# mihikamd/DP-GSAT

Measured on AMD Instinct MI355X. Metric: million edges/s (attn+sample+aggregate fwd+bwd), higher is better.
Workload: dtype f32

## Files before the change

### dp_gsat_amd/csrc/pna.hip

```cpp
#include "common.h"
#include "pna_math.h"

namespace gsat {

constexpr int PNA_BLOCK = 128;
constexpr int SC_AMP = GSAT_SCALE_AMPLIFICATION, SC_ATT = GSAT_SCALE_ATTENUATION, SC_LIN = GSAT_SCALE_LINEAR, SC_INVLIN = GSAT_SCALE_INVERSE_LINEAR;

struct PnaCfg {
    int A, S;
    int aggr[8];
    int scal[8];
    float avg_lin, avg_log;
};

__device__ __forceinline__ int pna_xcd_remap(int b, int nb) {
    int q = nb >> 3, r = nb & 7, x = b & 7, i = b >> 3;
    return (x < r ? x * (q + 1) : r * (q + 1) + (x - r) * q) + i;
}

__device__ __forceinline__ float scaler_factor(int s, float deg, float avg_lin, float avg_log) {
    switch (s) {
        case SC_AMP: return logf(deg + 1.f) / avg_log;
        case SC_ATT: return deg == 0.f ? 1.f : avg_log / logf(deg + 1.f);
        case SC_LIN: return deg / avg_lin;
// ... 539 lines not shown
                const int k = kb + u, e = e4[u];
                const float w = w4[u];
                const float4 xj = x4[u];
                float da = 0.f;
                if (on) {
                    float4 dm;
                    dm.x = fmaf(Qj.x, w * xj.x, Pj.x) + (k == jmin.x ? gmn_j.x : 0.f) + (k == jmax.x ? gmx_j.x : 0.f);
                    dm.y = fmaf(Qj.y, w * xj.y, Pj.y) + (k == jmin.y ? gmn_j.y : 0.f) + (k == jmax.y ? gmx_j.y : 0.f);
                    dm.z = fmaf(Qj.z, w * xj.z, Pj.z) + (k == jmin.z ? gmn_j.z : 0.f) + (k == jmax.z ? gmx_j.z : 0.f);
                    dm.w = fmaf(Qj.w, w * xj.w, Pj.w) + (k == jmin.w ? gmn_j.w : 0.f) + (k == jmax.w ? gmx_j.w : 0.f);
                    st4(dmsg + (size_t)k * H + c, f4scale(w, dm));
                    da += f4dot(dm, xj);
                    da += t1 + w * t2 + (k == kmin_a ? tmn : 0.f) + (k == kmax_a ? tmx : 0.f);
                    if (HAS_EE) {
                        const float4 ee = ee4[u];
                        float4 de;
                        de.x = fmaf(Qe.x, w * ee.x, Pe.x) + (k == emin.x ? gmn_e.x : 0.f) + (k == emax.x ? gmx_e.x : 0.f);
                        de.y = fmaf(Qe.y, w * ee.y, Pe.y) + (k == emin.y ? gmn_e.y : 0.f) + (k == emax.y ? gmx_e.y : 0.f);
                        de.z = fmaf(Qe.z, w * ee.z, Pe.z) + (k == emin.z ? gmn_e.z : 0.f) + (k == emax.z ? gmx_e.z : 0.f);
                        de.w = fmaf(Qe.w, w * ee.w, Pe.w) + (k == emin.w ? gmn_e.w : 0.f) + (k == emax.w ? gmx_e.w : 0.f);
                        if (dedge) st4(dedge + (size_t)e * H + c, f4scale(w, de));
                        da += f4dot(de, ee);
                    }
                }
                if (datt) {
                    da = group_sum<LPR>(da);
                    if (lane == 0) datt[e] = c0 ? datt[e] + da : da;
                }
            }
        }
    }
}

constexpr int TILE_BLOCK = 512;

__global__ void k_pna_tiles(const int32_t* __restrict__ node_ptr, const int32_t* __restrict__ node_seg, const int32_t* __restrict__ rowptr,
                            const int32_t* __restrict__ rowptr_src, int N, int TN, int slack, int T, int4* __restrict__ desc,
                            int32_t* __restrict__ spill_count) {
    const int t = blockIdx.x * blockDim.x + threadIdx.x;
    if (t == 0 && spill_count) *spill_count = 0;
    if (t > T) return;
    const int64_t p = (int64_t)t * TN;
    int start = N;
    if (t < T && p < N) {
        start = (int)p;
        if (node_seg) {
            const int g0 = node_ptr[node_seg[p]];
            start = min((int)p, max(g0, (int)p - slack));
        }
    }
    desc[t] = make_int4(start, rowptr[start], rowptr_src[start], 0);
}

template <int LPR, int NAGG, bool NATT>
__global__ __launch_bounds__(TILE_BLOCK, 4) void k_pna_bwd_tile(
    const float* __restrict__ x, const float* __restrict__ att, const float* __restrict__ dout, const int32_t* __restrict__ rowptr,
    const int32_t* __restrict__ col, const int32_t* __restrict__ eid, const int4* __restrict__ desc,
    const int32_t* __restrict__ rowptr_src, const int32_t* __restrict__ slot_map, int H, int TE, int RCAP, float* dx,
    float* __restrict__ dmsg, float* datt, float* __restrict__ dw, const float* __restrict__ dx_add, int datt_acc) {
    constexpr int GPB = LaneGroups<LPR, TILE_BLOCK>::GPB;
    constexpr int RPW = 64 / LPR;
    constexpr int NSEG = NAGG * 2;
    extern __shared__ float4 smem4[];
    float4* erow = smem4;
    int* s_col = reinterpret_cast<int*>(erow + (size_t)TE * LPR);
    int* s_eid = s_col + TE;
    float* s_w = reinterpret_cast<float*>(s_eid);
    float* s_att = reinterpret_cast<float*>(s_eid + TE);
    int* s_slot = reinterpret_cast<int*>(s_att + TE);
    int* s_rp = s_slot + TE;
    int* s_rps = s_rp + RCAP + 1;
    float* s_na = reinterpret_cast<float*>(s_rps + RCAP + 1);
    float* s_dna = s_na + RCAP + 1;
    const int tid = threadIdx.x, wave = tid >> 6;
    const LaneGroups<LPR, TILE_BLOCK> lg;
    const int grp = lg.grp < 0 ? GPB : lg.grp;
    const int lane = lg.lane, c = lane * 4;
    const bool on = c < H && lg.grp >= 0;
    const int t = pna_xcd_remap(blockIdx.x, gridDim.x);
    const int4 d0 = desc[t], d1 = desc[t + 1];
    const int n0 = d0.x, n1 = d1.x;
    if (n1 <= n0) return;
    const int nr = n1 - n0;
    const int k0 = d0.y, ne = min(d1.y - k0, TE);
    const int s0 = d0.z, ns = d1.z - s0, nsl = min(ns, TE);
    float4 dcur[NSEG];
    float4 xi_cur = f4zero();
    const uint32_t hb = (uint32_t)H * 4u, gb = NSEG * hb, cb = (uint32_t)c * 4u;
    const float* gwin = dout + (size_t)n0 * NSEG * H;
    const float* xwin = x + (size_t)n0 * H;
    float* dxwin = dx + (size_t)n0 * H;
    float* mwin = dmsg + (size_t)k0 * H;
    int r = lg.grp >= 0 ? grp : nr;
#pragma unroll
    for (int sg = 0; sg < NSEG; ++sg) dcur[sg] = f4zero();
    if (r < nr && on) {
#pragma unroll
        for (int sg = 0; sg < NSEG; ++sg) dcur[sg] = ld4_off(gwin, r * gb + sg * hb + cb);
        xi_cur = ld4_off(xwin, r * hb + cb);
    }
    for (int i = tid; i <= nr; i += TILE_BLOCK) {
        s_rp[i] = rowptr[n0 + i] - k0;
        s_rps[i] = rowptr_src[n0 + i] - s0;
        if (NATT) { s_na[i] = att[min(n0 + i, n1 - 1)]; s_dna[i] = 0.f; }
    }
    for (int i = tid; i < ne; i += TILE_BLOCK) {
        s_col[i] = col[k0 + i];
        if (!NATT) s_eid[i] = eid[k0 + i];
    }
    for (int i = tid; i < nsl; i += TILE_BLOCK) s_slot[i] = slot_map[s0 + i] - k0;
    __syncthreads();
    for (int base = 0; base < ne; base += GPB) {
        const int i = base + grp;
        if (i < ne && on)
            __builtin_amdgcn_global_load_lds((const __attribute__((address_space(1))) void*)(x + (size_t)s_col[i] * H + c),
                                             (__attribute__((address_space(3))) void*)(erow + (size_t)(base + wave * RPW) * LPR), 16, 0, 0);
    }
    for (int i = tid; i < ne; i += TILE_BLOCK) {
        if (NATT) {
            s_att[i] = att[s_col[i]];
        } else {
            s_att[i] = att ? att[s_eid[i]] : 1.f;
        }
    }
    asm volatile("s_waitcnt vmcnt(0)" ::: "memory");
    __syncthreads();
    float4 dx_keep = f4zero();
    for (; r < nr; r += GPB) {
        const int nr_ = r + GPB;
        const int beg = s_rp[r], end = s_rp[r + 1];
        const float na_row = NATT ? s_na[r] : 0.f;
        const float cnt = (float)(end - beg);
        float sa = 0.f, sa2 = 0.f, amin = INFINITY, amax = -INFINITY;
        int kmin_a = beg, kmax_a = beg;
        Acc4 aj;
        aj.init();
        int4 jmin = make_int4(beg, beg, beg, beg), jmax = jmin;
        float wfirst = 1.f;
        const int mid = min(end, max(beg, ne));
        auto stats = [&](int k, float w, float4 xv) {
            if (k == beg) wfirst = w;
            sa += w; sa2 = fmaf(w, w, sa2);
            if (w < amin) { amin = w; kmin_a = k; }
            if (w > amax) { amax = w; kmax_a = k; }
            const float4 m = f4scale(w, xv);
#define GSAT_TARG(C)                                                                                                       \
            if (m.C < aj.mn.C) { jmin.C = k; aj.mn.C = m.C; }                                                              \
            if (m.C > aj.mx.C) { jmax.C = k; aj.mx.C = m.C; }
            GSAT_TARG(x) GSAT_TARG(y) GSAT_TARG(z) GSAT_TARG(w)
#undef GSAT_TARG
            aj.s.x += m.x; aj.s.y += m.y; aj.s.z += m.z; aj.s.w += m.w;
            aj.q.x = fmaf(m.x, m.x, aj.q.x); aj.q.y = fmaf(m.y, m.y, aj.q.y); aj.q.z = fmaf(m.z, m.z, aj.q.z); aj.q.w = fmaf(m.w, m.w, aj.q.w);
        };
        for (int k = beg; k < mid; ++k)
            stats(k, NATT ? s_att[k] * na_row : s_att[k], on ? erow[(size_t)k * LPR + lane] : f4zero());
        for (int k = mid; k < end; ++k)
            stats(k, NATT ? att[col[k0 + k]] * na_row : (att ? att[eid[k0 + k]] : 1.f), on ? ld4(x + (size_t)col[k0 + k] * H + c) : f4zero());
        const float4 xi = xi_cur;
        const Acc4 ai = self_stats(xi, sa, sa2, amin, amax);
        const float n = fmaxf(cnt, 1.f), inv_n = 1.f / n;
        float t1 = 0.f, t2 = 0.f, tmn = 0.f, tmx = 0.f;
        float4 Pi, Qi, Pj, Qj, gmn_i, gmx_i, gmn_j, gmx_j;
#define GSAT_TFOLD(ACC, PART, P, Q, GMN, GMX)                                                                              \
        {                                                                                                                  \
            const float4 mean = f4scale(inv_n, ACC.s);                                                                     \
            const float4 var = make_float4(ACC.q.x * inv_n - mean.x * mean.x, ACC.q.y * inv_n - mean.y * mean.y,           \
                                           ACC.q.z * inv_n - mean.z * mean.z, ACC.q.w * inv_n - mean.w * mean.w);          \
            const float4 hs = make_float4(var.x > 0.f ? 0.5f * __builtin_amdgcn_rsqf(var.x + 1e-5f) : 0.f,                 \
                                          var.y > 0.f ? 0.5f * __builtin_amdgcn_rsqf(var.y + 1e-5f) : 0.f,                 \
                                          var.z > 0.f ? 0.5f * __builtin_amdgcn_rsqf(var.z + 1e-5f) : 0.f,                 \
                                          var.w > 0.f ? 0.5f * __builtin_amdgcn_rsqf(var.w + 1e-5f) : 0.f);                \
            float4 p0 = f4scale(inv_n, dcur[0 * 2 + (PART)]);                                                              \
            if (NAGG == 5) { const float4 vsum = dcur[(NAGG == 5 ? 4 : 0) * 2 + (PART)];                                   \
                             p0 = make_float4(p0.x + vsum.x, p0.y + vsum.y, p0.z + vsum.z, p0.w + vsum.w); }               \
            GMN = dcur[1 * 2 + (PART)];                                                                                    \
            GMX = dcur[2 * 2 + (PART)];                                                                                    \
            const float4 vs = dcur[3 * 2 + (PART)];                                                                        \
            const float4 gv = make_float4(vs.x * hs.x, vs.y * hs.y, vs.z * hs.z, vs.w * hs.w);                             \
            Q = f4scale(2.f * inv_n, gv);                                                                                  \
            P = make_float4(p0.x - mean.x * Q.x, p0.y - mean.y * Q.y, p0.z - mean.z * Q.z, p0.w - mean.w * Q.w);           \
        }
        GSAT_TFOLD(ai, 0, Pi, Qi, gmn_i, gmx_i)
        if (on) {
            float4 dxi;
#define GSAT_TSELF(C)                                                                                                      \
            {                                                                                                              \
                const float xc = xi.C;                                                                                     \
                const float wlo = xc > 0.f ? amin : (xc < 0.f ? amax : wfirst), whi = xc > 0.f ? amax : (xc < 0.f ? amin : wfirst); \
                dxi.C = Pi.C * sa + Qi.C * xc * sa2 + gmn_i.C * wlo + gmx_i.C * whi;                                       \
                t1 = fmaf(Pi.C, xc, t1);                                                                                   \
                t2 = fmaf(Qi.C * xc, xc, t2);                                                                              \
                tmn += xc > 0.f ? gmn_i.C * xc : (xc < 0.f ? gmx_i.C * xc : 0.f);                                          \
                tmx += xc > 0.f ? gmx_i.C * xc : (xc < 0.f ? gmn_i.C * xc : 0.f);                                          \
            }
            GSAT_TSELF(x) GSAT_TSELF(y) GSAT_TSELF(z) GSAT_TSELF(w)
#undef GSAT_TSELF
            if (end == beg) dxi = f4zero();
            if (nr_ < nr) st4_off(dxwin, r * hb + cb, dxi); else dx_keep = dxi;
        }
        GSAT_TFOLD(aj, 1, Pj, Qj, gmn_j, gmx_j)
#undef GSAT_TFOLD
        if (nr_ < nr && on) {
#pragma unroll
            for (int sg = 0; sg < NSEG; ++sg) dcur[sg] = ld4_off(gwin, nr_ * gb + sg * hb + cb);
            xi_cur = ld4_off(xwin, nr_ * hb + cb);
        }
        float dna_acc = 0.f;
        auto grad = [&](int k, float w, float a_src, int j, int e, float4 xj, bool lds) {
            const bool in_lds = lds && j >= n0 && j < n1;
            float da = 0.f;
            if (on) {
                float4 dm;
                dm.x = fmaf(Qj.x, w * xj.x, Pj.x) + (k == jmin.x ? gmn_j.x : 0.f) + (k == jmax.x ? gmx_j.x : 0.f);
                dm.y = fmaf(Qj.y, w * xj.y, Pj.y) + (k == jmin.y ? gmn_j.y : 0.f) + (k == jmax.y ? gmx_j.y : 0.f);
                dm.z = fmaf(Qj.z, w * xj.z, Pj.z) + (k == jmin.z ? gmn_j.z : 0.f) + (k == jmax.z ? gmx_j.z : 0.f);
                dm.w = fmaf(Qj.w, w * xj.w, Pj.w) + (k == jmin.w ? gmn_j.w : 0.f) + (k == jmax.w ? gmx_j.w : 0.f);
                const float4 o = f4scale(w, dm);
                if (in_lds) st4_lds(erow + (size_t)k * LPR + lane, o);
                else if (lds) st4_off(mwin, k * hb + cb, o);
                else st4(dmsg + (size_t)(k0 + k) * H + c, o);
                da = f4dot(dm, xj) + t1 + w * t2 + (k == kmin_a ? tmn : 0.f) + (k == kmax_a ? tmx : 0.f);
            }
            if (datt) {
                da = group_sum<LPR>(da);
                if (NATT) {
                    if (lane == 0) {
                        dna_acc = fmaf(da, a_src, dna_acc);
                        const float share = da * na_row;
                        if (in_lds) st1_lds(s_w + k, share); else dw[k0 + k] = share;
                    }
                } else if (lane == 0) datt[e] = da;
            }
        };
        for (int k = beg; k < mid; ++k) {
            const float a = s_att[k];
            grad(k, NATT ? a * na_row : a, a, s_col[k], NATT ? 0 : s_eid[k], on ? erow[(size_t)k * LPR + lane] : f4zero(), true);
        }
        for (int k = mid; k < end; ++k) {
            const int j = col[k0 + k], e = NATT ? 0 : eid[k0 + k];
            const float a = NATT ? att[j] : (att ? att[e] : 1.f);
            grad(k, NATT ? a * na_row : a, a, j, e, on ? ld4(x + (size_t)j * H + c) : f4zero(), false);
        }
        if (NATT && datt && lane == 0) s_dna[r] = dna_acc;
    }
    __syncthreads();
    const float* awin = dx_add ? dx_add + (size_t)n0 * H : nullptr;
    for (int j = lg.grp >= 0 ? grp : nr; j < nr; j += GPB) {
        if (!on) continue;
        const int sb = s_rps[j], se = s_rps[j + 1];
        float4 acc = j + GPB < nr ? ld4_off(dxwin, j * hb + cb) : dx_keep;
        const float dprev = (NATT && datt && datt_acc && lane == 0) ? datt[n0 + j] : 0.f;
        if (awin) {
            const float4 ra = ld4_off(awin, j * hb + cb);
            acc.x += ra.x; acc.y += ra.y; acc.z += ra.z; acc.w += ra.w;
        }
        float sw = 0.f;
        for (int s_ = sb; s_ < se; ++s_) {
            const int kl = s_ < nsl ? s_slot[s_] : slot_map[s0 + s_] - k0;
            if (kl >= 0 && kl < ne) {
                const float4 v = erow[(size_t)kl * LPR + lane];
                acc.x += v.x; acc.y += v.y; acc.z += v.z; acc.w += v.w;
                if (NATT && datt) sw += s_w[kl];
            }
        }
        st4_off(dxwin, j * hb + cb, acc);
        if (NATT && datt && lane == 0) datt[n0 + j] = (s_dna[j] + sw) + dprev;
    }
}

__global__ void k_pna_spill_rows(const int4* __restrict__ desc, int TN, int TE, const int32_t* __restrict__ rowptr_src,
                                 const int32_t* __restrict__ slot_map, int num_rows, int32_t* __restrict__ spill_rows,
                                 int32_t* __restrict__ spill_count) {
    const int j = blockIdx.x * blockDim.x + threadIdx.x;
    if (j >= num_rows) return;
    const int sb = rowptr_src[j], se = rowptr_src[j + 1];
    if (sb == se) return;
    int t = j / TN;
    if (j >= desc[t + 1].x) ++t;
    const int k0 = desc[t].y, ne = min(desc[t + 1].y - k0, TE);
    bool flag = false;
    for (int s_ = sb; s_ < se && !flag; ++s_) {
        const int k = slot_map[s_];
        flag = k < k0 || k >= k0 + ne;
    }
    if (flag) {
        const int idx = atomicAdd(spill_count, 1);
        if (idx < num_rows) spill_rows[idx] = j;
    }
}

template <int LPR>
__global__ __launch_bounds__(256) void k_pna_bwd_spill(const float* __restrict__ dmsg, const int4* __restrict__ desc, int TN, int TE,
                                                       const int32_t* __restrict__ rowptr_src, const int32_t* __restrict__ slot_map,
                                                       const int32_t* __restrict__ spill_rows, const int32_t* __restrict__ spill_count,
                                                       int num_rows, int H, float* __restrict__ dx, const float* __restrict__ dw,
                                                       float* __restrict__ dna) {
    const LaneGroups<LPR, 256> lg;
    constexpr int GPB = LaneGroups<LPR, 256>::GPB;
    const int lane = lg.lane, c = lane * 4;
    const int count = min(*spill_count, num_rows);
    if (lg.grp < 0) return;
    for (int i = blockIdx.x * GPB + lg.grp; i < count; i += gridDim.x * GPB) {
        const int j = spill_rows[i];
        const int sb = rowptr_src[j], se = rowptr_src[j + 1];
        int t = j / TN;
        if (j >= desc[t + 1].x) ++t;
        const int k0 = desc[t].y, ne = min(desc[t + 1].y - k0, TE);
        if (c >= H) continue;
        float4 acc = ld4(dx + (size_t)j * H + c);
        float sw = 0.f;
        for (int s_ = sb; s_ < se; ++s_) {
            const int k = slot_map[s_];
            if (k >= k0 && k < k0 + ne) continue;
            const float4 v = ld4(dmsg + (size_t)k * H + c);
            acc.x += v.x; acc.y += v.y; acc.z += v.z; acc.w += v.w;
            if (dna) sw += dw[k];
        }
        st4(dx + (size_t)j * H + c, acc);
        if (dna && lane == 0) dna[j] += sw;
    }
}

static inline int pna_lpr(int64_t H) {
    if (H <= 0 || H % 4 != 0 || H > 256) return 0;
    int64_t q = H / 4;
    return q <= 4 ? 4 : q <= 8 ? 8 : q <= 16 ? 16 : q <= 20 ? 20 : q <= 32 ? 32 : 64;
}

constexpr int PNA_CHUNK = 256;
static inline bool pna_width_ok(int64_t H) { return H > 0 && H % 4 == 0 && H <= 512; }

static inline void pna_grid(int64_t N, int lpr, int* nb, int* rpg) {
    const int gpb = (PNA_BLOCK / 64) * (64 / lpr);
    int64_t b = ceil_div(N, gpb);
    if (b > 256 * 64) b = 256 * 64;
    if (b < 1) b = 1;
    *nb = (int)b;
    *rpg = (int)std::max<int64_t>(1, ceil_div(N, b * gpb));
}

static inline int fixed_aggregators(const PnaCfg& cfg) {
    if (cfg.S != 1 || cfg.scal[0] != 0 || (cfg.A != 4 && cfg.A != 5)) return 0;
    if (cfg.aggr[0] != AGG_MEAN || cfg.aggr[1] != AGG_MIN || cfg.aggr[2] != AGG_MAX || cfg.aggr[3] != GSAT_AGG_STD) return 0;
    if (cfg.A == 5 && cfg.aggr[4] != AGG_SUM) return 0;
    return cfg.A;
}

static int make_cfg(const int32_t* aggr, int A, const int32_t* scal, int S, float avg_lin, float avg_log, PnaCfg* cfg) {
    GSAT_REQUIRE(aggr && scal && A >= 1 && A <= 8 && S >= 1 && S <= 8, GSAT_ERR_ARG, "pna: need 1..8 aggregators and scalers");
    cfg->A = A; cfg->S = S; cfg->avg_lin = avg_lin; cfg->avg_log = avg_log;
    for (int i = 0; i < 8; ++i) { cfg->aggr[i] = 0; cfg->scal[i] = 0; }
    for (int i = 0; i < A; ++i) {
        GSAT_REQUIRE(aggr[i] >= 0 && aggr[i] <= 5, GSAT_ERR_ARG, "pna: unknown aggregator code %d", aggr[i]);
        cfg->aggr[i] = aggr[i];
    }
    for (int i = 0; i < S; ++i) {
        GSAT_REQUIRE(scal[i] >= 0 && scal[i] <= 4, GSAT_ERR_ARG, "pna: unknown scaler code %d", scal[i]);
        cfg->scal[i] = scal[i];
    }
    return GSAT_OK;
}

template <int L, int NA, bool NATT>
static hipError_t pna_tile_allow_lds(size_t lds) {
    static size_t allowed = 0;
    if (lds <= allowed) return hipSuccess;
    hipError_t e = hipFuncSetAttribute((const void*)k_pna_bwd_tile<L, NA, NATT>, hipFuncAttributeMaxDynamicSharedMemorySize, (int)lds);
    if (e == hipSuccess) allowed = lds;
    return e;
}

static size_t pna_tile_lds_bytes(int lpr, int edges_cap, int rows_cap) {
    return (size_t)edges_cap * ((size_t)lpr * 16 + 16) + (size_t)(rows_cap + 1) * 16;
}

}

using namespace gsat;

#define GSAT_LPR_DISPATCH(lpr, CALL) \
    switch (lpr) { case 4: CALL(4); break; case 8: CALL(8); break; case 16: CALL(16); break; case 20: CALL(20); break; case 32: CALL(32); break; default: CALL(64); break; }

extern "C" {

static int pna_fwd_impl(const char* who, const float* x, const float* att, const float* edge_emb, const int32_t* rowptr, const int32_t* col,
                        const int32_t* eid, int64_t N, int64_t E, int64_t H, const int32_t* aggregators, int A, const int32_t* scalers, int S,
                        float avg_deg_lin, float avg_deg_log, float* out, const int32_t* chunk_ptr, float* partial, hipStream_t stream,
                        float* scal_out = nullptr) {
    GSAT_REQUIRE(N >= 0 && N < (1ll << 31), GSAT_ERR_ARG, "%s: bad N", who);
    PnaCfg cfg;
    int rc = make_cfg(aggregators, A, scalers, S, avg_deg_lin, avg_deg_log, &cfg);
    if (rc) return rc;
    if (N == 0) return GSAT_OK;
    GSAT_REQUIRE(pna_width_ok(H), GSAT_ERR_UNSUPPORTED, "%s: H=%lld must be a multiple of 4 and <= 512", who, (long long)H);
    GSAT_REQUIRE(x && rowptr && out, GSAT_ERR_ARG, "%s: null pointer", who);
    GSAT_REQUIRE(chunk_ptr == nullptr || partial != nullptr, GSAT_ERR_ARG, "%s: chunk_ptr needs the record workspace", who);
    if (E <= CH) chunk_ptr = nullptr;
    const int nagg = fixed_aggregators(cfg);
    GSAT_REQUIRE(!scal_out || (nagg && !edge_emb && !chunk_ptr), GSAT_ERR_UNSUPPORTED,
                 "%s: the compact output needs (mean,min,max,std[,sum]) with the identity scaler, no edge features, no hub chunks", who);
    for (int c0 = 0; c0 < (int)H; c0 += PNA_CHUNK) {
        const int Hc = std::min<int>(PNA_CHUNK, (int)H - c0);
        const int lpr = pna_lpr(Hc);
        int nb, rpg;
        pna_grid(N, lpr, &nb, &rpg);
        const int gpb = (PNA_BLOCK / 64) * (64 / lpr);
        const int cb = chunk_ptr ? (int)std::min<int64_t>(ceil_div(pna_max_chunks(E), gpb), 256 * 16) : 0;
#define GO(L, EE, NA)                                                                                                                       \
    do {                                                                                                                                    \
        k_pna_fwd<L, EE, NA, false><<<nb, PNA_BLOCK, 0, stream>>>(x, att, edge_emb, rowptr, col, eid, (int)N, (int)H, cfg, out, rpg, c0, Hc, chunk_ptr, partial, scal_out); \
        if (cb) k_pna_fwd<L, EE, NA, true><<<cb, PNA_BLOCK, 0, stream>>>(x, att, edge_emb, rowptr, col, eid, (int)N, (int)H, cfg, out, rpg, c0, Hc, chunk_ptr, partial, scal_out); \
    } while (0)
#define CALL(L)                                                                                                              \
    do {                                                                                                                     \
        if (edge_emb) {                                                                                                      \
            if (cb) k_pna_chunk_stats<L, true><<<cb, PNA_BLOCK, 0, stream>>>(x, att, edge_emb, rowptr, col, eid, (int)N, (int)H, chunk_ptr, partial, c0, Hc); \
            if (nagg == 4) GO(L, true, 4); else if (nagg == 5) GO(L, true, 5); else GO(L, true, 0);                          \
        } else {                                                                                                             \
            if (cb) k_pna_chunk_stats<L, false><<<cb, PNA_BLOCK, 0, stream>>>(x, att, edge_emb, rowptr, col, eid, (int)N, (int)H, chunk_ptr, partial, c0, Hc); \
            if (nagg == 4) GO(L, false, 4); else if (nagg == 5) GO(L, false, 5); else GO(L, false, 0);                       \
        }                                                                                                                    \
    } while (0)
// ... 110 lines not shown
    if (lds_budget_bytes <= 0) lds_budget_bytes = 80 * 1024;
    GSAT_REQUIRE(lds_budget_bytes <= 160 * 1024, GSAT_ERR_ARG, "gsat_pna_tile_plan: LDS budget above 160 KiB");
    int64_t te = (lds_budget_bytes - 64) / ((int64_t)lpr * 16 + 16 + 8);
    te = te / 8 * 8;
    GSAT_REQUIRE(te >= 16, GSAT_ERR_UNSUPPORTED, "gsat_pna_tile_plan: LDS budget too small for H=%lld", (long long)H);
    int64_t half = std::max<int64_t>(4, te / 4 / 4 * 4);
    *rows_nominal = (int32_t)half;
    *rows_slack = (int32_t)half;
    *edges_cap = (int32_t)te;
    return GSAT_OK;
}

int gsat_pna_build_tiles(const int32_t* node_ptr, const int32_t* node_seg, const int32_t* rowptr, const int32_t* rowptr_src,
                         const int32_t* slot_dst_of_srcslot, int64_t N, int rows_nominal, int rows_slack, int edges_cap, int32_t* tile_desc,
                         int32_t* spill_rows, int32_t* spill_count, void* stream_) {
    hipStream_t stream = (hipStream_t)stream_;
    GSAT_REQUIRE(N >= 0 && N < (1ll << 31) && rows_nominal > 0 && rows_slack >= 0 && rows_slack <= rows_nominal && tile_desc && rowptr && rowptr_src,
                 GSAT_ERR_ARG, "gsat_pna_build_tiles: bad argument");
    GSAT_REQUIRE(((uintptr_t)tile_desc & 15) == 0, GSAT_ERR_ARG, "gsat_pna_build_tiles: tile_desc must be 16-byte aligned");
    GSAT_REQUIRE((node_ptr == nullptr) == (node_seg == nullptr), GSAT_ERR_ARG, "gsat_pna_build_tiles: node_ptr and node_seg go together");
    const int64_t T = ceil_div(N, rows_nominal);
    k_pna_tiles<<<(int)ceil_div(T + 1, 256), 256, 0, stream>>>(node_ptr, node_seg, rowptr, rowptr_src, (int)N, rows_nominal, node_seg ? rows_slack : 0, (int)T,
                                                               (int4*)tile_desc, spill_count);
    GSAT_LAUNCH_CHECK();
    GSAT_REQUIRE(spill_rows && spill_count && edges_cap > 0, GSAT_ERR_ARG, "gsat_pna_build_tiles: null spill list");
    if (N > 0 && slot_dst_of_srcslot) {
        k_pna_spill_rows<<<(int)ceil_div(N, 256), 256, 0, stream>>>((const int4*)tile_desc, rows_nominal, edges_cap, rowptr_src, slot_dst_of_srcslot,
                                                                   (int)N, spill_rows, spill_count);
        GSAT_LAUNCH_CHECK();
    }
    return GSAT_OK;
}

static int pna_bwd_tiled_impl(const char* who, bool natt, const float* x, const float* att, const float* dout, const int32_t* rowptr,
                              const int32_t* col, const int32_t* eid, const int32_t* tile_desc, int64_t num_tiles, int rows_nominal,
                              int rows_cap, int edges_cap, const int32_t* rowptr_src, const int32_t* slot_dst_of_srcslot, int64_t N,
                              int64_t E, int64_t H, const int32_t* aggregators, int A, const int32_t* scalers, int S,
                              const int32_t* spill_rows, const int32_t* spill_count, float* dx, float* dmsg, float* datt, float* dw,
                              const float* dx_add, int datt_acc, hipStream_t stream) {
    GSAT_REQUIRE(N >= 0 && N < (1ll << 31) && E >= 0 && num_tiles >= 0, GSAT_ERR_ARG, "%s: bad extents", who);
    PnaCfg cfg;
    int rc = make_cfg(aggregators, A, scalers, S, 1.f, 1.f, &cfg);
    if (rc) return rc;
    const int nagg = fixed_aggregators(cfg);
    GSAT_REQUIRE(nagg, GSAT_ERR_UNSUPPORTED, "%s: only (mean,min,max,std[,sum]) with the identity scaler", who);
    if (N == 0) return GSAT_OK;
    const int lpr = pna_lpr(H);
    GSAT_REQUIRE(lpr, GSAT_ERR_UNSUPPORTED, "%s: H=%lld must be a multiple of 4 and <= 256", who, (long long)H);
    GSAT_REQUIRE(x && dout && rowptr && tile_desc && rowptr_src && dx && rows_nominal > 0 && rows_cap >= rows_nominal && rows_cap <= 2 * rows_nominal && edges_cap > 0, GSAT_ERR_ARG, "%s: null pointer", who);
    GSAT_REQUIRE(E == 0 || (col && (natt || eid) && slot_dst_of_srcslot && dmsg), GSAT_ERR_ARG, "%s: null edge arrays", who);
    GSAT_REQUIRE(!natt || (att && (!datt || dw || E == 0)), GSAT_ERR_ARG, "%s: node attention needs node_att and, for its gradient, the [E] scratch dw", who);
    const size_t lds = pna_tile_lds_bytes(lpr, edges_cap, rows_cap);
    GSAT_REQUIRE(lds <= 160 * 1024, GSAT_ERR_ARG, "%s: tile needs %zu bytes of LDS", who, lds);
#define GO(L, NA, NT)                                                                                                        \
    do {                                                                                                                     \
        GSAT_CHECK_HIP((pna_tile_allow_lds<L, NA, NT>(lds)));                                                                \
        k_pna_bwd_tile<L, NA, NT><<<(int)num_tiles, TILE_BLOCK, lds, stream>>>(x, att, dout, rowptr, col, eid, (const int4*)tile_desc,     \
                                                                          rowptr_src, slot_dst_of_srcslot, (int)H, edges_cap, rows_cap, dx, dmsg, datt, dw, dx_add, datt_acc); \
    } while (0)
#define CALL(L) do { if (natt) { if (nagg == 4) GO(L, 4, true); else GO(L, 5, true); } else { if (nagg == 4) GO(L, 4, false); else GO(L, 5, false); } } while (0)
    if (num_tiles > 0) { GSAT_LPR_DISPATCH(lpr, CALL); }
#undef CALL
#undef GO
    GSAT_LAUNCH_CHECK();
    if (E > 0) {
        GSAT_REQUIRE(spill_rows && spill_count, GSAT_ERR_ARG, "%s: null spill list (gsat_pna_build_tiles)", who);
        const int nb = (int)std::min<int64_t>(std::max<int64_t>(ceil_div(N, 8 * 4 * (64 / lpr)), 1), 256 * 8);
        const float* dw_in = (natt && datt) ? dw : nullptr;
        float* dna = (natt && datt) ? datt : nullptr;
#define CALL(L) k_pna_bwd_spill<L><<<nb, 256, 0, stream>>>(dmsg, (const int4*)tile_desc, rows_nominal, edges_cap, rowptr_src, slot_dst_of_srcslot, spill_rows, spill_count, (int)N, (int)H, dx, dw_in, dna)
        GSAT_LPR_DISPATCH(lpr, CALL);
#undef CALL
        GSAT_LAUNCH_CHECK();
    }
    return GSAT_OK;
}

int gsat_pna_bwd_tiled(const float* x, const float* att, const float* dout, const int32_t* rowptr, const int32_t* col,
                       const int32_t* eid, const int32_t* tile_desc, int64_t num_tiles, int rows_nominal, int rows_cap, int edges_cap,
                       const int32_t* rowptr_src, const int32_t* slot_dst_of_srcslot, int64_t N, int64_t E, int64_t H,
                       const int32_t* aggregators, int A, const int32_t* scalers, int S, const int32_t* spill_rows,
                       const int32_t* spill_count, float* dx, float* dmsg, float* datt, const float* dx_add, void* stream_) {
    return pna_bwd_tiled_impl("gsat_pna_bwd_tiled", false, x, att, dout, rowptr, col, eid, tile_desc, num_tiles, rows_nominal, rows_cap, edges_cap,
                              rowptr_src, slot_dst_of_srcslot, N, E, H, aggregators, A, scalers, S, spill_rows, spill_count, dx, dmsg, datt,
                              nullptr, dx_add, 0, (hipStream_t)stream_);
}

int gsat_pna_bwd_tiled_node_att(const float* x, const float* node_att, const float* dout, const int32_t* rowptr, const int32_t* col,
                                const int32_t* tile_desc, int64_t num_tiles, int rows_nominal, int rows_cap, int edges_cap,
                                const int32_t* rowptr_src, const int32_t* slot_dst_of_srcslot, int64_t N, int64_t E, int64_t H,
                                const int32_t* aggregators, int A, const int32_t* scalers, int S, const int32_t* spill_rows,
                                const int32_t* spill_count, float* dx, float* dmsg, float* dnode_att, float* dw, const float* dx_add,
                                int accumulate_dnode_att, void* stream_) {
    return pna_bwd_tiled_impl("gsat_pna_bwd_tiled_node_att", true, x, node_att, dout, rowptr, col, nullptr, tile_desc, num_tiles, rows_nominal,
                              rows_cap, edges_cap, rowptr_src, slot_dst_of_srcslot, N, E, H, aggregators, A, scalers, S, spill_rows, spill_count,
                              dx, dmsg, dnode_att, dw, dx_add, accumulate_dnode_att, (hipStream_t)stream_);
}

}
```

Baseline: 124.8.

## Make PNA backward tile kernel persistent with prefetch of next tile metadata

After: 119.9. 0.961x the previous value.

```diff
diff --git a/dp_gsat_amd/csrc/pna.hip b/dp_gsat_amd/csrc/pna.hip
--- a/dp_gsat_amd/csrc/pna.hip
+++ b/dp_gsat_amd/csrc/pna.hip
@@ -615,11 +615,22 @@
     desc[t] = make_int4(start, rowptr[start], rowptr_src[start], 0);
 }
 
+#ifdef GSAT_PNA_TILE_STAMPS
+constexpr int TILE_STAMP_WGS = 8192;
+__device__ unsigned long long g_pna_tile_stamps[TILE_STAMP_WGS][8];
+#define GSAT_TILE_STAMP_INIT long long st_[6] = {0, 0, 0, 0, 0, 0}; asm volatile("" ::: "memory"); long long stl_ = __builtin_amdgcn_s_memtime();
+#define GSAT_TILE_STAMP(i) { asm volatile("s_waitcnt lgkmcnt(0)" ::: "memory"); if (threadIdx.x == 0) { const long long n_ = __builtin_amdgcn_s_memtime(); st_[i] += n_ - stl_; stl_ = n_; if ((i) == 4) ++st_[5]; } }
+#define GSAT_TILE_STAMP_FLUSH if (threadIdx.x == 0 && blockIdx.x < TILE_STAMP_WGS) { for (int i_ = 0; i_ < 6; ++i_) g_pna_tile_stamps[blockIdx.x][i_] += (unsigned long long)st_[i_]; }
+#else
+#define GSAT_TILE_STAMP_INIT
+#define GSAT_TILE_STAMP(i)
+#define GSAT_TILE_STAMP_FLUSH
+#endif
 template <int LPR, int NAGG, bool NATT>
 __global__ __launch_bounds__(TILE_BLOCK, 4) void k_pna_bwd_tile(
     const float* __restrict__ x, const float* __restrict__ att, const float* __restrict__ dout, const int32_t* __restrict__ rowptr,
     const int32_t* __restrict__ col, const int32_t* __restrict__ eid, const int4* __restrict__ desc,
-    const int32_t* __restrict__ rowptr_src, const int32_t* __restrict__ slot_map, int H, int TE, int RCAP, float* dx,
+    const int32_t* __restrict__ rowptr_src, const int32_t* __restrict__ slot_map, int H, int TE, int RCAP, int T, float* dx,
     float* __restrict__ dmsg, float* datt, float* __restrict__ dw, const float* __restrict__ dx_add, int datt_acc) {
     constexpr int GPB = LaneGroups<LPR, TILE_BLOCK>::GPB;
     constexpr int RPW = 64 / LPR;
@@ -635,200 +646,274 @@
     int* s_rps = s_rp + RCAP + 1;
     float* s_na = reinterpret_cast<float*>(s_rps + RCAP + 1);
     float* s_dna = s_na + RCAP + 1;
-    const int tid = threadIdx.x, wave = tid >> 6;
+    const int tid0 = threadIdx.x;
     const LaneGroups<LPR, TILE_BLOCK> lg;
     const int grp = lg.grp < 0 ? GPB : lg.grp;
     const int lane = lg.lane, c = lane * 4;
     const bool on = c < H && lg.grp >= 0;
-    const int t = pna_xcd_remap(blockIdx.x, gridDim.x);
-    const int4 d0 = desc[t], d1 = desc[t + 1];
-    const int n0 = d0.x, n1 = d1.x;
-    if (n1 <= n0) return;
-    const int nr = n1 - n0;
-    const int k0 = d0.y, ne = min(d1.y - k0, TE);
-    const int s0 = d0.z, ns = d1.z - s0, nsl = min(ns, TE);
     float4 dcur[NSEG];
-    float4 xi_cur = f4zero();
+    float4 xi_cur;
     const uint32_t hb = (uint32_t)H * 4u, gb = NSEG * hb, cb = (uint32_t)c * 4u;
-    const float* gwin = dout + (size_t)n0 * NSEG * H;
-    const float* xwin = x + (size_t)n0 * H;
-    float* dxwin = dx + (size_t)n0 * H;
-    float* mwin = dmsg + (size_t)k0 * H;
-    int r = lg.grp >= 0 ? grp : nr;
-#pragma unroll
-    for (int sg = 0; sg < NSEG; ++sg) dcur[sg] = f4zero();
-    if (r < nr && on) {
-#pragma unroll
-        for (int sg = 0; sg < NSEG; ++sg) dcur[sg] = ld4_off(gwin, r * gb + sg * hb + cb);
-        xi_cur = ld4_off(xwin, r * hb + cb);
-    }
-    for (int i = tid; i <= nr; i += TILE_BLOCK) {
-        s_rp[i] = rowptr[n0 + i] - k0;
-        s_rps[i] = rowptr_src[n0 + i] - s0;
-        if (NATT) { s_na[i] = att[min(n0 + i, n1 - 1)]; s_dna[i] = 0.f; }
-    }
-    for (int i = tid; i < ne; i += TILE_BLOCK) {
-        s_col[i] = col[k0 + i];
-        if (!NATT) s_eid[i] = eid[k0 + i];
-    }
-    for (int i = tid; i < nsl; i += TILE_BLOCK) s_slot[i] = slot_map[s0 + i] - k0;
-    __syncthreads();
-    for (int base = 0; base < ne; base += GPB) {
-        const int i = base + grp;
-        if (i < ne && on)
-            __builtin_amdgcn_global_load_lds((const __attribute__((address_space(1))) void*)(x + (size_t)s_col[i] * H + c),
-                                             (__attribute__((address_space(3))) void*)(erow + (size_t)(base + wave * RPW) * LPR), 16, 0, 0);
-    }
-    for (int i = tid; i < ne; i += TILE_BLOCK) {
-        if (NATT) {
-            s_att[i] = att[s_col[i]];
+    auto first_rows = [&](const int4 a, const int4 b) {
+#pragma unroll
+        for (int sg = 0; sg < NSEG; ++sg) dcur[sg] = f4zero();
+        xi_cur = f4zero();
+        int g = grp;
+        asm volatile("" : "+v"(g));
+        if (g < b.x - a.x && on) {
+            const float* gw = dout + (size_t)a.x * NSEG * H;
+            uint32_t off = g * gb + cb;
+#pragma unroll
+            for (int sg = 0; sg < NSEG; ++sg) { dcur[sg] = ld4_off(gw, off); off += hb; }
+            xi_cur = ld4_off(x + (size_t)a.x * H, g * hb + cb);
+        }
+    };
+    int p_rp = 0, p_rps = 0, p_col = 0, p_eid = 0, p_slot = 0;
+    float p_na = 0.f;
+    bool ahead = false;
+    GSAT_TILE_STAMP_INIT
+    int4 d0, d1, e0, e1;
+    {
+        const int t = pna_xcd_remap(blockIdx.x, T);
+        d0 = desc[t]; d1 = desc[t + 1];
+    }
+    GSAT_TILE_STAMP(0)
+    first_rows(d0, d1);
+    for (int v = blockIdx.x; v < T; v += gridDim.x, d0 = e0, d1 = e1) {
+        int tid = tid0;
+        asm volatile("" : "+v"(tid));
+        const int wave = tid >> 6;
+        const bool more = v + (int)gridDim.x < T;
+        e0 = d1; e1 = d1;
+        const int n0 = d0.x, n1 = d1.x;
+        if (n1 <= n0) {
+            ahead = false;
+            if (more) {
+                const int tn = pna_xcd_remap(v + gridDim.x, T);
+                e0 = desc[tn]; e1 = desc[tn + 1];
+                first_rows(e0, e1);
+            }
+            continue;
+        }
+        const int nr = n1 - n0;
+        const int k0 = d0.y, ne = min(d1.y - k0, TE);
+        const int s0 = d0.z, ns = d1.z - s0, nsl = min(ns, TE);
+        const float* gwin = dout + (size_t)n0 * NSEG * H;
+        const float* xwin = x + (size_t)n0 * H;
+        float* dxwin = dx + (size_t)n0 * H;
+        float* mwin = dmsg + (size_t)k0 * H;
+        int r = lg.grp >= 0 ? grp : nr;
+        if (ahead) {
+            if (tid <= nr) {
+                s_rp[tid] = p_rp;
+                s_rps[tid] = p_rps;
+                if (NATT) { s_na[tid] = p_na; s_dna[tid] = 0.f; }
+            }
+            if (tid < ne) {
+                s_col[tid] = p_col;
+                if (!NATT) s_eid[tid] = p_eid;
+            }
+            if (tid < nsl) s_slot[tid] = p_slot;
         } else {
-            s_att[i] = att ? att[s_eid[i]] : 1.f;
-        }
-    }
-    asm volatile("s_waitcnt vmcnt(0)" ::: "memory");
-    __syncthreads();
-    float4 dx_keep = f4zero();
-    for (; r < nr; r += GPB) {
-        const int nr_ = r + GPB;
-        const int beg = s_rp[r], end = s_rp[r + 1];
-        const float na_row = NATT ? s_na[r] : 0.f;
-        const float cnt = (float)(end - beg);
-        float sa = 0.f, sa2 = 0.f, amin = INFINITY, amax = -INFINITY;
-        int kmin_a = beg, kmax_a = beg;
-        Acc4 aj;
-        aj.init();
-        int4 jmin = make_int4(beg, beg, beg, beg), jmax = jmin;
-        float wfirst = 1.f;
-        const int mid = min(end, max(beg, ne));
-        auto stats = [&](int k, float w, float4 xv) {
-            if (k == beg) wfirst = w;
-            sa += w; sa2 = fmaf(w, w, sa2);
-            if (w < amin) { amin = w; kmin_a = k; }
-            if (w > amax) { amax = w; kmax_a = k; }
-            const float4 m = f4scale(w, xv);
+            for (int i = tid; i <= nr; i += TILE_BLOCK) {
+                s_rp[i] = rowptr[n0 + i] - k0;
+                s_rps[i] = rowptr_src[n0 + i] - s0;
+                if (NATT) { s_na[i] = att[min(n0 + i, n1 - 1)]; s_dna[i] = 0.f; }
+            }
+            for (int i = tid; i < ne; i += TILE_BLOCK) {
+                s_col[i] = col[k0 + i];
+                if (!NATT) s_eid[i] = eid[k0 + i];
+            }
+            for (int i = tid; i < nsl; i += TILE_BLOCK) s_slot[i] = slot_map[s0 + i] - k0;
+        }
+        __syncthreads();
+        GSAT_TILE_STAMP(1)
+        for (int base = 0; base < ne; base += GPB) {
+            const int i = base + grp;
+            if (i < ne && on)
+                __builtin_amdgcn_global_load_lds((const __attribute__((address_space(1))) void*)(x + (size_t)s_col[i] * H + c),
+                                                 (__attribute__((address_space(3))) void*)(erow + (size_t)(base + wave * RPW) * LPR), 16, 0, 0);
+        }
+        for (int i = tid; i < ne; i += TILE_BLOCK) {
+            if (NATT) {
+                s_att[i] = att[s_col[i]];
+            } else {
+                s_att[i] = att ? att[s_eid[i]] : 1.f;
+            }
+        }
+        asm volatile("s_waitcnt vmcnt(0)" ::: "memory");
+        __syncthreads();
+        GSAT_TILE_STAMP(2)
+        float4 dx_keep = f4zero();
+        for (; r < nr; r += GPB) {
+            const int nr_ = r + GPB;
+            const int beg = s_rp[r], end = s_rp[r + 1];
+            const float na_row = NATT ? s_na[r] : 0.f;
+            const float cnt = (float)(end - beg);
+            float sa = 0.f, sa2 = 0.f, amin = INFINITY, amax = -INFINITY;
+            int kmin_a = beg, kmax_a = beg;
+            Acc4 aj;
+            aj.init();
+            int4 jmin = make_int4(beg, beg, beg, beg), jmax = jmin;
+            float wfirst = 1.f;
+            const int mid = min(end, max(beg, ne));
+            auto stats = [&](int k, float w, float4 xv) {
+                if (k == beg) wfirst = w;
+                sa += w; sa2 = fmaf(w, w, sa2);
+                if (w < amin) { amin = w; kmin_a = k; }
+                if (w > amax) { amax = w; kmax_a = k; }
+                const float4 m = f4scale(w, xv);
 #define GSAT_TARG(C)                                                                                                       \
-            if (m.C < aj.mn.C) { jmin.C = k; aj.mn.C = m.C; }                                                              \
-            if (m.C > aj.mx.C) { jmax.C = k; aj.mx.C = m.C; }
-            GSAT_TARG(x) GSAT_TARG(y) GSAT_TARG(z) GSAT_TARG(w)
+                if (m.C < aj.mn.C) { jmin.C = k; aj.mn.C = m.C; }                                                              \
+                if (m.C > aj.mx.C) { jmax.C = k; aj.mx.C = m.C; }
+                GSAT_TARG(x) GSAT_TARG(y) GSAT_TARG(z) GSAT_TARG(w)
 #undef GSAT_TARG
-            aj.s.x += m.x; aj.s.y += m.y; aj.s.z += m.z; aj.s.w += m.w;
-            aj.q.x = fmaf(m.x, m.x, aj.q.x); aj.q.y = fmaf(m.y, m.y, aj.q.y); aj.q.z = fmaf(m.z, m.z, aj.q.z); aj.q.w = fmaf(m.w, m.w, aj.q.w);
-        };
-        for (int k = beg; k < mid; ++k)
-            stats(k, NATT ? s_att[k] * na_row : s_att[k], on ? erow[(size_t)k * LPR + lane] : f4zero());
-        for (int k = mid; k < end; ++k)
-            stats(k, NATT ? att[col[k0 + k]] * na_row : (att ? att[eid[k0 + k]] : 1.f), on ? ld4(x + (size_t)col[k0 + k] * H + c) : f4zero());
-        const float4 xi = xi_cur;
-        const Acc4 ai = self_stats(xi, sa, sa2, amin, amax);
-        const float n = fmaxf(cnt, 1.f), inv_n = 1.f / n;
-        float t1 = 0.f, t2 = 0.f, tmn = 0.f, tmx = 0.f;
-        float4 Pi, Qi, Pj, Qj, gmn_i, gmx_i, gmn_j, gmx_j;
+                aj.s.x += m.x; aj.s.y += m.y; aj.s.z += m.z; aj.s.w += m.w;
+                aj.q.x = fmaf(m.x, m.x, aj.q.x); aj.q.y = fmaf(m.y, m.y, aj.q.y); aj.q.z = fmaf(m.z, m.z, aj.q.z); aj.q.w = fmaf(m.w, m.w, aj.q.w);
+            };
+            for (int k = beg; k < mid; ++k)
+                stats(k, NATT ? s_att[k] * na_row : s_att[k], on ? erow[(size_t)k * LPR + lane] : f4zero());
+            for (int k = mid; k < end; ++k)
+                stats(k, NATT ? att[col[k0 + k]] * na_row : (att ? att[eid[k0 + k]] : 1.f), on ? ld4(x + (size_t)col[k0 + k] * H + c) : f4zero());
+            const float4 xi = xi_cur;
+            const Acc4 ai = self_stats(xi, sa, sa2, amin, amax);
+            const float n = fmaxf(cnt, 1.f), inv_n = 1.f / n;
+            float t1 = 0.f, t2 = 0.f, tmn = 0.f, tmx = 0.f;
+            float4 Pi, Qi, Pj, Qj, gmn_i, gmx_i, gmn_j, gmx_j;
 #define GSAT_TFOLD(ACC, PART, P, Q, GMN, GMX)                                                                              \
-        {                                                                                                                  \
-            const float4 mean = f4scale(inv_n, ACC.s);                                                                     \
-            const float4 var = make_float4(ACC.q.x * inv_n - mean.x * mean.x, ACC.q.y * inv_n - mean.y * mean.y,           \
-                                           ACC.q.z * inv_n - mean.z * mean.z, ACC.q.w * inv_n - mean.w * mean.w);          \
-            const float4 hs = make_float4(var.x > 0.f ? 0.5f * __builtin_amdgcn_rsqf(var.x + 1e-5f) : 0.f,                 \
-                                          var.y > 0.f ? 0.5f * __builtin_amdgcn_rsqf(var.y + 1e-5f) : 0.f,                 \
-                                          var.z > 0.f ? 0.5f * __builtin_amdgcn_rsqf(var.z + 1e-5f) : 0.f,                 \
-                                          var.w > 0.f ? 0.5f * __builtin_amdgcn_rsqf(var.w + 1e-5f) : 0.f);                \
-            float4 p0 = f4scale(inv_n, dcur[0 * 2 + (PART)]);                                                              \
-            if (NAGG == 5) { const float4 vsum = dcur[(NAGG == 5 ? 4 : 0) * 2 + (PART)];                                   \
-                             p0 = make_float4(p0.x + vsum.x, p0.y + vsum.y, p0.z + vsum.z, p0.w + vsum.w); }               \
-            GMN = dcur[1 * 2 + (PART)];                                                                                    \
-            GMX = dcur[2 * 2 + (PART)];                                                                                    \
-            const float4 vs = dcur[3 * 2 + (PART)];                                                                        \
-            const float4 gv = make_float4(vs.x * hs.x, vs.y * hs.y, vs.z * hs.z, vs.w * hs.w);                             \
-            Q = f4scale(2.f * inv_n, gv);                                                                                  \
-            P = make_float4(p0.x - mean.x * Q.x, p0.y - mean.y * Q.y, p0.z - mean.z * Q.z, p0.w - mean.w * Q.w);           \
-        }
-        GSAT_TFOLD(ai, 0, Pi, Qi, gmn_i, gmx_i)
-        if (on) {
-            float4 dxi;
+            {                                                                                                                  \
+                const float4 mean = f4scale(inv_n, ACC.s);                                                                     \
+                const float4 var = make_float4(ACC.q.x * inv_n - mean.x * mean.x, ACC.q.y * inv_n - mean.y * mean.y,           \
+                                               ACC.q.z * inv_n - mean.z * mean.z, ACC.q.w * inv_n - mean.w * mean.w);          \
+                const float4 hs = make_float4(var.x > 0.f ? 0.5f * __builtin_amdgcn_rsqf(var.x + 1e-5f) : 0.f,                 \
+                                              var.y > 0.f ? 0.5f * __builtin_amdgcn_rsqf(var.y + 1e-5f) : 0.f,                 \
+                                              var.z > 0.f ? 0.5f * __builtin_amdgcn_rsqf(var.z + 1e-5f) : 0.f,                 \
+                                              var.w > 0.f ? 0.5f * __builtin_amdgcn_rsqf(var.w + 1e-5f) : 0.f);                \
+                float4 p0 = f4scale(inv_n, dcur[0 * 2 + (PART)]);                                                              \
+                if (NAGG == 5) { const float4 vsum = dcur[(NAGG == 5 ? 4 : 0) * 2 + (PART)];                                   \
+                                 p0 = make_float4(p0.x + vsum.x, p0.y + vsum.y, p0.z + vsum.z, p0.w + vsum.w); }               \
+                GMN = dcur[1 * 2 + (PART)];                                                                                    \
+                GMX = dcur[2 * 2 + (PART)];                                                                                    \
+                const float4 vs = dcur[3 * 2 + (PART)];                                                                        \
+                const float4 gv = make_float4(vs.x * hs.x, vs.y * hs.y, vs.z * hs.z, vs.w * hs.w);                             \
+                Q = f4scale(2.f * inv_n, gv);                                                                                  \
+                P = make_float4(p0.x - mean.x * Q.x, p0.y - mean.y * Q.y, p0.z - mean.z * Q.z, p0.w - mean.w * Q.w);           \
+            }
+            GSAT_TFOLD(ai, 0, Pi, Qi, gmn_i, gmx_i)
+            if (on) {
+                float4 dxi;
 #define GSAT_TSELF(C)                                                                                                      \
-            {                                                                                                              \
-                const float xc = xi.C;                                                                                     \
-                const float wlo = xc > 0.f ? amin : (xc < 0.f ? amax : wfirst), whi = xc > 0.f ? amax : (xc < 0.f ? amin : wfirst); \
-                dxi.C = Pi.C * sa + Qi.C * xc * sa2 + gmn_i.C * wlo + gmx_i.C * whi;                                       \
-                t1 = fmaf(Pi.C, xc, t1);                                                                                   \
-                t2 = fmaf(Qi.C * xc, xc, t2);                                                                              \
-                tmn += xc > 0.f ? gmn_i.C * xc : (xc < 0.f ? gmx_i.C * xc : 0.f);                                          \
-                tmx += xc > 0.f ? gmx_i.C * xc : (xc < 0.f ? gmn_i.C * xc : 0.f);                                          \
-            }
-            GSAT_TSELF(x) GSAT_TSELF(y) GSAT_TSELF(z) GSAT_TSELF(w)
+                {                                                                                                              \
+                    const float xc = xi.C;                                                                                     \
+                    const float wlo = xc > 0.f ? amin : (xc < 0.f ? amax : wfirst), whi = xc > 0.f ? amax : (xc < 0.f ? amin : wfirst); \
+                    dxi.C = Pi.C * sa + Qi.C * xc * sa2 + gmn_i.C * wlo + gmx_i.C * whi;                                       \
+                    t1 = fmaf(Pi.C, xc, t1);                                                                                   \
+                    t2 = fmaf(Qi.C * xc, xc, t2);                                                                              \
+                    tmn += xc > 0.f ? gmn_i.C * xc : (xc < 0.f ? gmx_i.C * xc : 0.f);                                          \
+                    tmx += xc > 0.f ? gmx_i.C * xc : (xc < 0.f ? gmn_i.C * xc : 0.f);                                          \
+                }
+                GSAT_TSELF(x) GSAT_TSELF(y) GSAT_TSELF(z) GSAT_TSELF(w)
 #undef GSAT_TSELF
-            if (end == beg) dxi = f4zero();
-            if (nr_ < nr) st4_off(dxwin, r * hb + cb, dxi); else dx_keep = dxi;
-        }
-        GSAT_TFOLD(aj, 1, Pj, Qj, gmn_j, gmx_j)
+                if (end == beg) dxi = f4zero();
+                if (nr_ < nr) st4_off(dxwin, r * hb + cb, dxi); else dx_keep = dxi;
+            }
+            GSAT_TFOLD(aj, 1, Pj, Qj, gmn_j, gmx_j)
 #undef GSAT_TFOLD
-        if (nr_ < nr && on) {
-#pragma unroll
-            for (int sg = 0; sg < NSEG; ++sg) dcur[sg] = ld4_off(gwin, nr_ * gb + sg * hb + cb);
-            xi_cur = ld4_off(xwin, nr_ * hb + cb);
-        }
-        float dna_acc = 0.f;
-        auto grad = [&](int k, float w, float a_src, int j, int e, float4 xj, bool lds) {
-            const bool in_lds = lds && j >= n0 && j < n1;
-            float da = 0.f;
-            if (on) {
-                float4 dm;
-                dm.x = fmaf(Qj.x, w * xj.x, Pj.x) + (k == jmin.x ? gmn_j.x : 0.f) + (k == jmax.x ? gmx_j.x : 0.f);
-                dm.y = fmaf(Qj.y, w * xj.y, Pj.y) + (k == jmin.y ? gmn_j.y : 0.f) + (k == jmax.y ? gmx_j.y : 0.f);
-                dm.z = fmaf(Qj.z, w * xj.z, Pj.z) + (k == jmin.z ? gmn_j.z : 0.f) + (k == jmax.z ? gmx_j.z : 0.f);
-                dm.w = fmaf(Qj.w, w * xj.w, Pj.w) + (k == jmin.w ? gmn_j.w : 0.f) + (k == jmax.w ? gmx_j.w : 0.f);
-                const float4 o = f4scale(w, dm);
-                if (in_lds) st4_lds(erow + (size_t)k * LPR + lane, o);
-                else if (lds) st4_off(mwin, k * hb + cb, o);
-                else st4(dmsg + (size_t)(k0 + k) * H + c, o);
-                da = f4dot(dm, xj) + t1 + w * t2 + (k == kmin_a ? tmn : 0.f) + (k == kmax_a ? tmx : 0.f);
-            }
-            if (datt) {
-                da = group_sum<LPR>(da);
-                if (NATT) {
-                    if (lane == 0) {
-                        dna_acc = fmaf(da, a_src, dna_acc);
-                        const float share = da * na_row;
-                        if (in_lds) st1_lds(s_w + k, share); else dw[k0 + k] = share;
-                    }
-                } else if (lane == 0) datt[e] = da;
-            }
-        };
-        for (int k = beg; k < mid; ++k) {
-            const float a = s_att[k];
-            grad(k, NATT ? a * na_row : a, a, s_col[k], NATT ? 0 : s_eid[k], on ? erow[(size_t)k * LPR + lane] : f4zero(), true);
-        }
-        for (int k = mid; k < end; ++k) {
-            const int j = col[k0 + k], e = NATT ? 0 : eid[k0 + k];
-            const float a = NATT ? att[j] : (att ? att[e] : 1.f);
-            grad(k, NATT ? a * na_row : a, a, j, e, on ? ld4(x + (size_t)j * H + c) : f4zero(), false);
-        }
-        if (NATT && datt && lane == 0) s_dna[r] = dna_acc;
-    }
-    __syncthreads();
-    const float* awin = dx_add ? dx_add + (size_t)n0 * H : nullptr;
-    for (int j = lg.grp >= 0 ? grp : nr; j < nr; j += GPB) {
-        if (!on) continue;
-        const int sb = s_rps[j], se = s_rps[j + 1];
-        float4 acc = j + GPB < nr ? ld4_off(dxwin, j * hb + cb) : dx_keep;
-        const float dprev = (NATT && datt && datt_acc && lane == 0) ? datt[n0 + j] : 0.f;
-        if (awin) {
-            const float4 ra = ld4_off(awin, j * hb + cb);
-            acc.x += ra.x; acc.y += ra.y; acc.z += ra.z; acc.w += ra.w;
-        }
-        float sw = 0.f;
-        for (int s_ = sb; s_ < se; ++s_) {
-            const int kl = s_ < nsl ? s_slot[s_] : slot_map[s0 + s_] - k0;
-            if (kl >= 0 && kl < ne) {
-                const float4 v = erow[(size_t)kl * LPR + lane];
-                acc.x += v.x; acc.y += v.y; acc.z += v.z; acc.w += v.w;
-                if (NATT && datt) sw += s_w[kl];
-            }
-        }
-        st4_off(dxwin, j * hb + cb, acc);
-        if (NATT && datt && lane == 0) datt[n0 + j] = (s_dna[j] + sw) + dprev;
-    }
+            if (nr_ < nr && on) {
+                uint32_t off = nr_ * gb + cb;
+                asm volatile("" : "+v"(off));
+#pragma unroll
+                for (int sg = 0; sg < NSEG; ++sg) { dcur[sg] = ld4_off(gwin, off); off += hb; }
+                xi_cur = ld4_off(xwin, nr_ * hb + cb);
+            }
+            float dna_acc = 0.f;
+            auto grad = [&](int k, float w, float a_src, int j, int e, float4 xj, bool lds) {
+                const bool in_lds = lds && j >= n0 && j < n1;
+                float da = 0.f;
+                if (on) {
+                    float4 dm;
+                    dm.x = fmaf(Qj.x, w * xj.x, Pj.x) + (k == jmin.x ? gmn_j.x : 0.f) + (k == jmax.x ? gmx_j.x : 0.f);
+                    dm.y = fmaf(Qj.y, w * xj.y, Pj.y) + (k == jmin.y ? gmn_j.y : 0.f) + (k == jmax.y ? gmx_j.y : 0.f);
+                    dm.z = fmaf(Qj.z, w * xj.z, Pj.z) + (k == jmin.z ? gmn_j.z : 0.f) + (k == jmax.z ? gmx_j.z : 0.f);
+                    dm.w = fmaf(Qj.w, w * xj.w, Pj.w) + (k == jmin.w ? gmn_j.w : 0.f) + (k == jmax.w ? gmx_j.w : 0.f);
+                    const float4 o = f4scale(w, dm);
+                    if (in_lds) st4_lds(erow + (size_t)k * LPR + lane, o);
+                    else if (lds) st4_off(mwin, k * hb + cb, o);
+                    else st4(dmsg + (size_t)(k0 + k) * H + c, o);
+                    da = f4dot(dm, xj) + t1 + w * t2 + (k == kmin_a ? tmn : 0.f) + (k == kmax_a ? tmx : 0.f);
+                }
+                if (datt) {
+                    da = group_sum<LPR>(da);
+                    if (NATT) {
+                        if (lane == 0) {
+                            dna_acc = fmaf(da, a_src, dna_acc);
+                            const float share = da * na_row;
+                            if (in_lds) st1_lds(s_w + k, share); else dw[k0 + k] = share;
+                        }
+                    } else if (lane == 0) datt[e] = da;
+                }
+            };
+            for (int k = beg; k < mid; ++k) {
+                const float a = s_att[k];
+                grad(k, NATT ? a * na_row : a, a, s_col[k], NATT ? 0 : s_eid[k], on ? erow[(size_t)k * LPR + lane] : f4zero(), true);
+            }
+            for (int k = mid; k < end; ++k) {
+                const int j = col[k0 + k], e = NATT ? 0 : eid[k0 + k];
+                const float a = NATT ? att[j] : (att ? att[e] : 1.f);
+                grad(k, NATT ? a * na_row : a, a, j, e, on ? ld4(x + (size_t)j * H + c) : f4zero(), false);
+            }
+            if (NATT && datt && lane == 0) s_dna[r] = dna_acc;
+        }
+        __syncthreads();
+        GSAT_TILE_STAMP(3)
+        ahead = false;
+        p_rp = p_rps = p_col = p_eid = p_slot = 0;
+        p_na = 0.f;
+        if (more) {
+            const int tn = pna_xcd_remap(v + gridDim.x, T);
+            e0 = desc[tn]; e1 = desc[tn + 1];
+            first_rows(e0, e1);
+            const int m0 = e0.x, mr = e1.x - m0, q0 = e0.y, qe = min(e1.y - q0, TE), z0 = e0.z, zs = min(e1.z - z0, TE);
+            ahead = mr > 0 && mr < TILE_BLOCK && qe <= TILE_BLOCK && zs <= TILE_BLOCK;
+            if (ahead) {
+                if (tid <= mr) {
+                    p_rp = rowptr[m0 + tid] - q0;
+                    p_rps = rowptr_src[m0 + tid] - z0;
+                    if (NATT) p_na = att[min(m0 + tid, e1.x - 1)];
+                }
+                if (tid < qe) {
+                    p_col = col[q0 + tid];
+                    if (!NATT) p_eid = eid[q0 + tid];
+                }
+                if (tid < zs) p_slot = slot_map[z0 + tid] - q0;
+            }
+        }
+        const float* awin = dx_add ? dx_add + (size_t)n0 * H : nullptr;
+        for (int j = lg.grp >= 0 ? grp : nr; j < nr; j += GPB) {
+            if (!on) continue;
+            const int sb = s_rps[j], se = s_rps[j + 1];
+            float4 acc = j + GPB < nr ? ld4_off(dxwin, j * hb + cb) : dx_keep;
+            const float dprev = (NATT && datt && datt_acc && lane == 0) ? datt[n0 + j] : 0.f;
+            if (awin) {
+                const float4 ra = ld4_off(awin, j * hb + cb);
+                acc.x += ra.x; acc.y += ra.y; acc.z += ra.z; acc.w += ra.w;
+            }
+            float sw = 0.f;
+            for (int s_ = sb; s_ < se; ++s_) {
+                const int kl = s_ < nsl ? s_slot[s_] : slot_map[s0 + s_] - k0;
+                if (kl >= 0 && kl < ne) {
+                    const float4 v = erow[(size_t)kl * LPR + lane];
+                    acc.x += v.x; acc.y += v.y; acc.z += v.z; acc.w += v.w;
+                    if (NATT && datt) sw += s_w[kl];
+                }
+            }
+            st4_off(dxwin, j * hb + cb, acc);
+            if (NATT && datt && lane == 0) datt[n0 + j] = (s_dna[j] + sw) + dprev;
+        }
+        __syncthreads();
+        GSAT_TILE_STAMP(4)
+    }
+    GSAT_TILE_STAMP_FLUSH
 }
 
 __global__ void k_pna_spill_rows(const int4* __restrict__ desc, int TN, int TE, const int32_t* __restrict__ rowptr_src,
@@ -931,6 +1016,24 @@
     hipError_t e = hipFuncSetAttribute((const void*)k_pna_bwd_tile<L, NA, NATT>, hipFuncAttributeMaxDynamicSharedMemorySize, (int)lds);
     if (e == hipSuccess) allowed = lds;
     return e;
+}
+
+template <int L, int NA, bool NATT>
+static hipError_t pna_tile_resident(size_t lds, int* wgs) {
+    static size_t asked = 0;
+    static int resident = 0;
+    if (lds != asked || resident <= 0) {
+        int per_cu = 0, dev = 0;
+        hipDeviceProp_t prop;
+        hipError_t e = hipOccupancyMaxActiveBlocksPerMultiprocessor(&per_cu, (const void*)k_pna_bwd_tile<L, NA, NATT>, TILE_BLOCK, lds);
+        if (e == hipSuccess) e = hipGetDevice(&dev);
+        if (e == hipSuccess) e = hipGetDeviceProperties(&prop, dev);
+        if (e != hipSuccess) return e;
+        resident = std::max(per_cu, 1) * std::max(prop.multiProcessorCount, 1);
+        asked = lds;
+    }
+    *wgs = resident;
+    return hipSuccess;
 }
 
 static size_t pna_tile_lds_bytes(int lpr, int edges_cap, int rows_cap) {
@@ -1147,11 +1250,18 @@
     GSAT_REQUIRE(!natt || (att && (!datt || dw || E == 0)), GSAT_ERR_ARG, "%s: node attention needs node_att and, for its gradient, the [E] scratch dw", who);
     const size_t lds = pna_tile_lds_bytes(lpr, edges_cap, rows_cap);
     GSAT_REQUIRE(lds <= 160 * 1024, GSAT_ERR_ARG, "%s: tile needs %zu bytes of LDS", who, lds);
+    GSAT_REQUIRE(num_tiles < (1ll << 31), GSAT_ERR_ARG, "%s: bad extents", who);
+    const char* env_grid = getenv("GSAT_PNA_TILE_GRID");
+    const int64_t want_grid = env_grid ? atoll(env_grid) : 0;
 #define GO(L, NA, NT)                                                                                                        \
     do {                                                                                                                     \
+        int grid = 0;                                                                                                        \
         GSAT_CHECK_HIP((pna_tile_allow_lds<L, NA, NT>(lds)));                                                                \
-        k_pna_bwd_tile<L, NA, NT><<<(int)num_tiles, TILE_BLOCK, lds, stream>>>(x, att, dout, rowptr, col, eid, (const int4*)tile_desc,     \
-                                                                          rowptr_src, slot_dst_of_srcslot, (int)H, edges_cap, rows_cap, dx, dmsg, datt, dw, dx_add, datt_acc); \
+        GSAT_CHECK_HIP((pna_tile_resident<L, NA, NT>(lds, &grid)));                                                          \
+        if (env_grid) grid = (int)std::min<int64_t>(std::max<int64_t>(want_grid, 1), num_tiles);                             \
+        grid = (int)std::min<int64_t>(grid, num_tiles);                                                                      \
+        k_pna_bwd_tile<L, NA, NT><<<grid, TILE_BLOCK, lds, stream>>>(x, att, dout, rowptr, col, eid, (const int4*)tile_desc,  \
+                                                                     rowptr_src, slot_dst_of_srcslot, (int)H, edges_cap, rows_cap, (int)num_tiles, dx, dmsg, datt, dw, dx_add, datt_acc); \
     } while (0)
 #define CALL(L) do { if (natt) { if (nagg == 4) GO(L, 4, true); else GO(L, 5, true); } else { if (nagg == 4) GO(L, 4, false); else GO(L, 5, false); } } while (0)
     if (num_tiles > 0) { GSAT_LPR_DISPATCH(lpr, CALL); }
@@ -1192,4 +1302,14 @@
                               dx, dmsg, dnode_att, dw, dx_add, accumulate_dnode_att, (hipStream_t)stream_);
 }
 
-}
+#ifdef GSAT_PNA_TILE_STAMPS
+int gsat_pna_tile_stamps(unsigned long long* out) {
+    GSAT_CHECK_HIP(hipDeviceSynchronize());
+    GSAT_CHECK_HIP(hipMemcpyFromSymbol(out, HIP_SYMBOL(g_pna_tile_stamps), sizeof(g_pna_tile_stamps)));
+    static unsigned long long zeros[TILE_STAMP_WGS][8];
+    GSAT_CHECK_HIP(hipMemcpyToSymbol(HIP_SYMBOL(g_pna_tile_stamps), zeros, sizeof(zeros)));
+    return GSAT_OK;
+}
+#endif
+
+}
```
